# pirovc/ganon

Measured on AMD Instinct MI355X. Metric: Mreads/s classified (150 bp) + IBF-lookup GB/s vs HBM roofline, higher is better.
Workload: dtype u64

## Files before the change

### ganon_amd/build.py

```python
from __future__ import annotations

import os
import shutil
import subprocess
import sys

HERE = os.path.dirname(os.path.abspath(__file__))
ROOT = os.path.dirname(HERE)
CSRC = os.path.join(HERE, "csrc")
HOST = os.path.join(HERE, "host")
LIB = os.path.join(CSRC, "libganon_hip.so")
BIN = os.path.join(HOST, "ganon-classify")
BIN_BUILD = os.path.join(HOST, "ganon-build")
BIN_REASSIGN = os.path.join(HOST, "ganon-reassign")
BUILD_SHARED = ("seq_io.cpp", "pgzip.cpp", "filter_io.cpp")
REASSIGN_ONLY = ("reassign.cpp", "reassign_main.cpp")

HIP_SOURCES = ["gn_kernels.hip", "gn_split.hip", "gn_minimiser_lpr.hip", "gn_hibf.hip", "gn_postfilter.hip", "gn_build.hip", "gn_build_hibf.hip", "gn_build_sketch.hip", "gn_gather.hip", "gn_fastq.hip", "gn_reassign.hip", "gn_inflate.hip", "gn_capi.hip"]
HIP_HEADERS = ["gn_internal.h", "gn_devmem.h", "gn_scan.h", "gn_build_row.h", "gn_bin_spans.h", "gn_fold_table.h", "gn_screen_table.h", "gn_emplace_window.h", "gn_packed_set.h", "gn_path_window.h", os.path.join(ROOT, "include", "ganon_hip.h"), os.path.join(ROOT, "include", "ganon_ibf_hash.h")]


def _hipcc() -> str:
    for c in (shutil.which("hipcc"), "/opt/rocm/bin/hipcc"):
        if c and os.path.exists(c):
            return c
    raise RuntimeError("hipcc not found: libganon_hip.so cannot be built (there is no CPU fallback)")


def _stale(target: str, deps) -> bool:
    if not os.path.exists(target):
        return True
    t = os.path.getmtime(target)
    return any(os.path.getmtime(d) > t for d in deps if os.path.exists(d))


def build_hip(force: bool = False, verbose: bool = False) -> str:
    import concurrent.futures as cf
    hdrs = [h if os.path.isabs(h) else os.path.join(CSRC, h) for h in HIP_HEADERS]
    objdir = os.path.join(CSRC, "_obj")
    os.makedirs(objdir, exist_ok=True)
    hipcc = None
    jobs, objs = [], []
    for s in HIP_SOURCES:
        src = os.path.join(CSRC, s)
        obj = os.path.join(objdir, os.path.splitext(s)[0] + ".o")
        objs.append(obj)
        if force or _stale(obj, [src] + hdrs):
            hipcc = hipcc or _hipcc()
            jobs.append([hipcc, "--offload-arch=gfx950", "-O3", "-std=c++17", "-fPIC", "-Wno-unused-result", "-Wno-unused-value",
                         "-c", src, "-o", obj])

    def run(cmd):
# ... 43 lines not shown
```

### ganon_amd/csrc/gn_capi.hip

```cpp
#include "gn_internal.h"

#include <hipcub/hipcub.hpp>
#include "gn_scan.h"
#include "gn_screen_table.h"

#include <algorithm>
#include <cstdarg>
#include <cstdio>
#include <cstdlib>
#include <cstring>
#include <mutex>
#include <new>
#include <unordered_map>
#include <vector>

#include <sys/mman.h>

static thread_local char g_err[512] = "";

int gn_fail(int code, const char* fmt, ...)
{
    va_list ap;
    va_start(ap, fmt);
    vsnprintf(g_err, sizeof(g_err), fmt, ap);
    va_end(ap);
    return code;
}

extern "C" const char* gn_last_error(void)
{
    return g_err;
}

static GnSwitches g_sw;

static int gn_parse_switches(const char* list, GnSwitches* out, char* bad, size_t bad_len)
{
    GnSwitches sw;
    struct
    {
        const char* name;
        bool GnSwitches::* flag;
    } static const flags[] = {{"early_exit", &GnSwitches::early_exit},       {"row_screen", &GnSwitches::row_screen},       {"lean_screen", &GnSwitches::lean_screen},     {"cand_select", &GnSwitches::cand_select},
                              {"csr_identity", &GnSwitches::csr_identity},   {"uniform_select", &GnSwitches::uniform_select},
                              {"run_select", &GnSwitches::run_select},       {"max_first", &GnSwitches::max_first},
                              {"const_nb", &GnSwitches::const_nb},           {"split_kernel", &GnSwitches::split_kernel},
                              {"predrop", &GnSwitches::predrop},             {"deferred_grids", &GnSwitches::deferred_grids}, {"on_demand", &GnSwitches::on_demand}, {"hibf_dense_rows", &GnSwitches::hibf_dense_rows},
                              {"hibf_reg", &GnSwitches::hibf_reg},           {"hibf_pack", &GnSwitches::hibf_pack},
                              {"hibf_one_pack", &GnSwitches::hibf_one_pack}, {"gather_copy", &GnSwitches::gather_copy},     {"joint_apart", &GnSwitches::joint_apart},
                              {"pinned_malloc", &GnSwitches::pinned_malloc}, {"inflate_ahead", &GnSwitches::inflate_ahead}, {"debug", &GnSwitches::debug},
                              {"fake_count", &GnSwitches::fake_count}, {"seg_result", &GnSwitches::seg_result}};
    for (const char* p = list ? list : ""; *p;)
    {
        const char* e = strchr(p, ',');
        size_t      n = e ? (size_t)(e - p) : strlen(p);
        while (n && (*p == ' ' || *p == '\t'))
            ++p, --n;
        while (n && (p[n - 1] == ' ' || p[n - 1] == '\t'))
            --n;
        bool known = n == 0;
        for (const auto& f : flags)
            if (!known && strlen(f.name) == n && !strncmp(p, f.name, n))
                sw.*(f.flag) = true, known = true;
        if (!known && n > 6 && !strncmp(p, "chunk=", 6))
            sw.chunk = (uint32_t)strtoul(p + 6, nullptr, 10), known = true;
        if (!known && n > 11 && !strncmp(p, "emit_probe=", 11))
            sw.emit_probe = (uint32_t)strtoul(p + 11, nullptr, 10) & (64u | 128u), known = true;
        if (!known && n > 16 && !strncmp(p, "hibf_pair_limit=", 16))
            sw.hibf_pair_limit = std::max<uint64_t>(64, strtoull(p + 16, nullptr, 10)), known = true;
        if (!known && n > 5 && !strncmp(p, "sync=", 5))
        {
            const char* m = p + 5;
            const size_t l = n - 5;
            sw.sync_mode = (l == 4 && !strncmp(m, "spin", 4)) ? 1 : (l == 5 && !strncmp(m, "yield", 5)) ? 2 : (l == 5 && !strncmp(m, "block", 5)) ? 3 : -1;
            known = sw.sync_mode > 0;
        }
// ... 1144 lines not shown
    p.hashes     = s->v_hashes;
    p.slot_off   = s->v_slot_off;
    p.n_hashes   = s->v_nh;
    p.status     = s->v_status;
    p.n_reads    = hi;
    p.read_begin = lo;
    p.rel_cutoff = s->rel_cutoff;
    if (gn_sw().fake_count)
    {
        if (lo == 0)
            s->pf_predrop = false;
        if ((uint64_t)(hi + 1) / 2 <= s->match_cap && hi > lo)
            hipLaunchKernelGGL(gn_fake_count_kernel, dim3((hi - lo + 255) / 256), dim3(256), 0, s->st, s->d_matches, s->d_seg_begin, s->d_seg_count,
                               s->v_status, s->v_nh, lo, hi, (uint32_t)f->geom.wpr, f->n_targets ? f->n_targets : 1u, s->d_ctr);
        GN_HIP(hipGetLastError());
        return GN_OK;
    }
    p.wpr        = f->geom.wpr;
    p.gp_log2    = f->geom.gp_log2;
    p.slice_dwords = f->geom.slice_dwords;
    p.matches    = s->d_matches;
    p.match_cap  = s->match_cap;
    p.cursor     = s->d_ctr;
    p.seg_begin  = s->d_seg_begin;
    p.seg_count  = s->d_seg_count;
    p.dense      = nullptr;
    p.max_blocks = (uint32_t)f->n_cu * 16u;
    p.max_blocks_fast = (uint32_t)f->n_cu * (f->geom.lw == 1 ? 8u : 6u);
    p.max_blocks_lean = (uint32_t)f->n_cu * 10u;
    p.max_blocks_list = p.max_blocks_fast;
    p.emit_probe = gn_sw().emit_probe;
    p.early_exit = gn_sw().early_exit ? 0u : 1u;
    p.skip_ctr   = s->d_ctr + 7;
    if (f->identity && p.early_exit && !gn_sw().row_screen && (f->geom.lw == 1 || p.W > 128))
    {
        uint8_t ds[GN_SCREEN_NMAX + 1];
        gn_screen_table(p.rel_cutoff, f->ibf.h, (uint32_t)std::min<uint64_t>(f->ibf.W, 64u * f->geom.lw) * 64u, ds);
        memcpy(p.screen, ds, sizeof(p.screen));
    }
    if (lo == 0)
        GN_HIP(hipMemsetAsync(s->d_ctr + 7, 0, sizeof(unsigned long long), s->st));
    p.sl_nbr = f->d_sl_nbr;
    p.csr_identity = f->csr_identity && !gn_sw().csr_identity ? 1u : 0u;
    p.uniform_nb   = p.csr_identity && !gn_sw().uniform_select ? f->uniform_nb : 0u;
    p.run_select   = p.csr_identity && f->run_ok && !p.uniform_nb && !gn_sw().run_select ? 1u : 0u;
    p.max_first    = gn_sw().max_first ? 0u : 1u;
    p.const_nb     = p.uniform_nb && !gn_sw().const_nb ? p.uniform_nb : (p.run_select ? 4u : 0u);
    const bool split = !f->identity && f->d_sl_nbr != nullptr && !gn_sw().split_kernel;
    const bool fast = f->identity;
    const bool predrop = (fast || split) && s->pf_on && !s->pf_merge && s->pf.d_segmin && s->pf_rel_filter >= 0.0 && s->pf_rel_filter < 1.0 &&
                         (uint64_t)hi * f->geom.wpr <= s->pf.segmin_cap && !gn_sw().predrop;
    if (lo == 0)
        s->pf_predrop = predrop;
    if (predrop)
    {
        if (lo == 0)
            GN_HIP(hipMemsetAsync(s->pf.d_pre, 0, sizeof(unsigned long long), s->st));
        GN_HIP(hipMemsetAsync(s->pf.d_segmin + (size_t)lo * f->geom.wpr, 0xFF, (size_t)(hi - lo) * f->geom.wpr * 4, s->st));
        p.pre_mode = s->pf_joint ? 2u : 1u;
        p.pre_rel  = s->pf_rel_filter;
        p.seg_min  = s->pf.d_segmin;
        p.pre_ctr  = s->pf.d_pre;
    }
    if (split)
    {
        GN_HIP(hipMemsetAsync(s->d_ctr + 4, 0, sizeof(unsigned long long), s->st));
// ... 640 lines not shown
```

### ganon_amd/csrc/gn_internal.h

```cpp
#pragma once

#include <hip/hip_runtime.h>
#include <stdint.h>

#include <vector>

#include "../../include/ganon_hip.h"
#include "../../include/ganon_ibf_hash.h"
#include "gn_devmem.h"
#include "gn_packed_set.h"

#define GN_MAX_CHUNKS 64
#define GN_CAND_NBIG 4u
#define GN_HIBF_MAXDEPTH 64
#define GN_HIBF_TIMED_LEVELS 8
#define GN_PF_MAX_JOINT 16
#define GN_PF_MAX_DEVICES 16
#define GN_LONG_BLOCKS 128u
#define GN_NCTR 74

struct GnSwitches
{
    bool early_exit = false;
    bool row_screen = false;
    bool lean_screen = false;
    bool cand_select = false;
    bool csr_identity = false;
    bool uniform_select = false;
    bool run_select = false;
    bool max_first = false;
    bool const_nb = false;
    bool split_kernel = false;
    bool predrop = false;
    bool deferred_grids = false;
    bool seg_result = false;
    bool on_demand = false;
    bool hibf_reg = false;
    bool hibf_pack = false;
    bool hibf_one_pack = false;
    bool hibf_dense_rows = false;
    bool     inflate_ahead = false;
    uint64_t hibf_pair_limit = 0;
    bool gather_copy = false;
    bool joint_apart = false;
    uint32_t chunk = 0;
    int      sync_mode = 0;
    bool     pinned_malloc = false;
    bool     debug = false;
    uint32_t emit_probe = 0;
    bool     fake_count = false;
};
const GnSwitches& gn_sw();
struct gn_stream;
int             gn_result_compact(gn_stream* s);
const gn_match* gn_result_matches(gn_stream* s);

struct GnMinimiserParams
{
// ... 41 lines not shown
    uint32_t wpr;
    uint32_t gp_log2;
    uint32_t slice_dwords;
    gn_match*           matches;
    uint64_t            match_cap;
    unsigned long long* cursor;
    uint64_t*           seg_begin;
    uint32_t*           seg_count;
    uint16_t* dense;
    uint32_t  dense_begin, dense_end;
    const uint32_t*           work_list;
    const unsigned long long* work_count;
    uint32_t*                 work_list_out;
    unsigned long long*       work_count_out;
    const uint32_t*           unit_list;
    const unsigned long long* unit_count;
    uint32_t*                 unit_list_out;
    unsigned long long*       unit_count_out;
    uint32_t                  max_blocks_lean;
    uint32_t                  max_blocks_list;
    uint32_t                  max_blocks;
    uint32_t                  max_blocks_fast;
    uint32_t                  emit_probe;
    const uint32_t*           bin_tgt;
    const uint32_t*           bin_nb2;
    uint32_t                  nbtab_off;
    uint32_t                  candcnt_off;
    const uint32_t*           big_list;
    uint32_t                  n_big;
    const uint32_t*           sl_nbr;
    uint32_t                  early_exit;
    unsigned long long*       skip_ctr;
    uint32_t                  screen[32];
    unsigned long long*       grab;
    uint32_t            uniform_nb;
    uint32_t            max_first;
    uint32_t            const_nb;
    uint32_t            run_select;
    uint32_t            csr_identity;
    uint32_t            pre_mode;
    double              pre_rel;
    uint32_t*           seg_min;
    unsigned long long* pre_ctr;
};

__device__ __forceinline__ uint32_t gn_pf_threshold(uint32_t mx, uint32_t mn, double rel_filter)
{
    return mx - (uint32_t)(unsigned long long)ceil(__dmul_rn((double)(mx - mn), rel_filter));
}

struct GnCountGeometry
{
    uint32_t lw;
    uint32_t wpr;
    uint32_t gp_log2;
    uint32_t block;
    uint32_t rpb;
    uint32_t slice_dwords;
    size_t   lds_bytes;
    size_t   nbtab_off;
    size_t   candcnt_off;
};

bool gn_count_geometry(uint64_t W, uint32_t hash_funs, GnCountGeometry* g, const char** why);
uint32_t gn_count_lds_index(const GnCountGeometry& g, uint32_t b);

// ... 269 lines not shown
```

### ganon_amd/csrc/gn_kernels.hip

```cpp
#include "gn_internal.h"
#include <cstdlib>

#define GN_WAVE 64
#define GN_CAND_LIMIT 128u
#ifndef GN_NARROW_MAX
#define GN_NARROW_MAX 4u
#endif
#define GN_MATCH_CHUNK 256u
#ifndef GN_MATCH_CHUNK_MAX
#define GN_MATCH_CHUNK_MAX 8192u
#endif
#define GN_STAGE_CAP 128u

struct GnRankLut
{
    uint8_t t[256];
    constexpr GnRankLut() : t{}
    {
        for (int i = 0; i < 256; ++i)
            t[i] = 0;
        t['C'] = t['c'] = 1;
        t['G'] = t['g'] = 2;
        t['T'] = t['t'] = t['U'] = t['u'] = 3;
        t['Y'] = t['y'] = 1;
        t['S'] = t['s'] = 1;
        t['K'] = t['k'] = 2;
        t['B'] = t['b'] = 1;
    }
};
__constant__ GnRankLut GN_RANK_LUT = GnRankLut();

__constant__ uint64_t GN_IBF_SEEDS[GN_IBF_MAX_HASH_FUNS] = GN_IBF_SEED_LIST;

__device__ __forceinline__ void gn_wave_lds_sync()
{
    __builtin_amdgcn_fence(__ATOMIC_RELEASE, "wavefront");
    __builtin_amdgcn_wave_barrier();
    __builtin_amdgcn_fence(__ATOMIC_ACQUIRE, "wavefront");
}

// ... 872 lines not shown
#ifndef GN_FAST_WPE_LW1
#define GN_FAST_WPE_LW1 4
#endif
#ifndef GN_FAST_WPE_LW2
#define GN_FAST_WPE_LW2 2
#endif
#ifndef GN_FAST_WPE_LW2_H4
#define GN_FAST_WPE_LW2_H4 3
#endif

constexpr uint32_t GN_FAST_EE_GP_LOG2 = 6;
static_assert((1u << GN_FAST_EE_GP_LOG2) == GN_WAVE, "the EE instances of the fast kernel: one hash group a wave");
template <int HF, int LW, bool EE, bool WIDE = false, bool SCRN = false>
__global__ __launch_bounds__(256) __attribute__((amdgpu_waves_per_eu(EE ? (LW == 1 ? GN_FAST_WPE_LW1 : (HF <= 4 && !WIDE ? GN_FAST_WPE_LW2_H4 : GN_FAST_WPE_LW2)) : 1))) void gn_ibf_count_fast_kernel(GnCountParams p)
{
    extern __shared__ __attribute__((aligned(16))) uint32_t gn_lds[];
    constexpr int      ND   = 2 * LW;
    constexpr int      HFP  = HF <= 4 ? 4 : 8;
    constexpr uint32_t NMAX = 127;
    constexpr bool     SCR  = SCRN && EE && HF == 4 && (LW == 1 || WIDE);
    static_assert(SCR == SCRN, "a screening instance: early exit, four hash functions, 8-byte lanes or the wide build");
    constexpr bool     LST  = EE && !SCRN && !WIDE && HF == 4 && LW == 1;

    const int      lane  = threadIdx.x & (GN_WAVE - 1);
    const int      wave  = __builtin_amdgcn_readfirstlane((int)(threadIdx.x >> 6));
    const uint32_t wpr   = p.wpr;
    const uint32_t gpl   = SCR ? GN_FAST_EE_GP_LOG2 : p.gp_log2;
    const uint32_t Gp    = 1u << gpl;
    const uint32_t H     = GN_WAVE >> gpl;
    const uint32_t gl    = lane & (Gp - 1);
    const uint32_t hsub  = lane >> gpl;
    uint32_t*      rowtab = gn_lds + (size_t)wave * 128 * HFP;
    uint32_t*      mlist  = gn_lds + (size_t)(blockDim.x >> 6) * 128 * HFP + (size_t)wave * GN_FAST_LIST;

    uint64_t       n_units = (uint64_t)(p.n_reads - p.read_begin) * wpr;
    if constexpr (LST)
        if (p.unit_list)
            n_units = *p.unit_count;
    const uint64_t stride  = (uint64_t)gridDim.x * (blockDim.x >> 6);
    uint64_t       unit    = (uint64_t)blockIdx.x * (blockDim.x >> 6) + wave;
    if (unit >= n_units)
        return;
    const bool     dyn      = p.grab != nullptr && n_units >= 64u * stride;
    const uint64_t dyn_from = stride * 16u;
    uint64_t       chunk_end = unit + 1;
    if (dyn)
    {
        unit *= 16u;
        chunk_end = unit + 16u;
    }
    unsigned long long g_next = 0;
    uint32_t           g_size = 16u;
    auto               ask    = [&](uint64_t from) {
        g_size = from < n_units - n_units / 4u ? 16u : (from < n_units - n_units / 16u ? 8u : 4u);
        if (lane == 0)
            g_next = atomicAdd(p.grab, (unsigned long long)g_size);
    };
    if (dyn)
        ask(unit);
    const uint32_t q0_c = (uint32_t)lane / HF, q1_c = ((uint32_t)lane + GN_WAVE) / HF;
    auto hash_of = [&](uint32_t& q0, uint32_t& q1) {
        if constexpr (!SCR)
        {
            q0 = q0_c;
            q1 = q1_c;
            return;
// ... 168 lines not shown
            const uint2 v = *reinterpret_cast<const uint2*>(ptr);
            R.m[i][0] = v.x;
            R.m[i][1] = v.y;
        }
    };
    bool scr = SCR && ds != 0;
    auto issue = [&](uint32_t it, GnRowRegs<HF, LW>& R) {
        uint32_t q = it * H + hsub;
        q          = q < n ? q : n - 1;
        uint32_t row[HF];
#pragma unroll
        for (int i = 0; i < HF; ++i)
        {
            uint32_t idx = q * HFP + (uint32_t)i;
            if constexpr (SCR)
            {
                const uint32_t qs = 2 * it + (uint32_t)(i >> 1) < ds ? 2 * it + (uint32_t)(i >> 1) : 2 * it;
                idx               = scr ? qs * HFP + (uint32_t)(i & 1) : idx;
            }
            row[i] = rowtab[idx];
        }
#pragma unroll
        for (int i = 0; i < HF; ++i)
            load_row(row[i], R, i);
    };
    auto consume = [&](const GnRowRegs<HF, LW>& R, uint32_t it) {
        if (SCR && scr)
        {
            const uint32_t on = col_act ? 0xFFFFFFFFu : 0u, on2 = 2 * it + 1 < ds ? on : 0u;
#pragma unroll
            for (int d = 0; d < ND; ++d)
            {
                const uint32_t a = R.m[0][d] & R.m[1][d] & on, b = R.m[2 % HF][d] & R.m[3 % HF][d] & on2;
#pragma unroll
                for (int j = 0; j < 4; ++j)
                    nib[d][j] += ((a >> j) & 0x11111111u) + ((b >> j) & 0x11111111u);
            }
            acc_n += 2;
            if (acc_n >= 14)
            {
                spill_nibbles();
                acc_n = 0;
            }
            return;
        }
        const uint32_t on = (col_act && it * H + hsub < n) ? 0xFFFFFFFFu : 0u;
#pragma unroll
        for (int d = 0; d < ND; ++d)
        {
            uint32_t a = R.m[0][d] & on;
#pragma unroll
            for (int i = 1; i < HF; ++i)
                a &= R.m[i][d];
#pragma unroll
            for (int j = 0; j < 4; ++j)
                nib[d][j] += (a >> j) & 0x11111111u;
        }
        if (++acc_n == 15)
        {
            spill_nibbles();
            acc_n = 0;
        }
    };
    uint32_t sm[ND];
#pragma unroll
    for (int d = 0; d < ND; ++d)
// ... 114 lines not shown
        scr_rows            = 2 * ds;
        const uint32_t left = survey(ds);
        if (left == 0)
            dead = true;
        else if (left <= GN_NARROW_MAX)
            finish = true;
        if (dead || finish)
            break;
        aborted = true;
#pragma unroll
        for (int d = 0; d < ND; ++d)
#pragma unroll
            for (int j = 0; j < 4; ++j)
            {
                byt[d][j][0] = 0;
                byt[d][j][1] = 0;
            }
        issue(0, A);
    }
    uint32_t narrow_loads = 0;
    if (EE && (narrow || (SCR && finish)))
    {
        constexpr uint32_t QPC = GN_WAVE / HF;
        uint64_t           grp = 0;
#pragma unroll
        for (uint32_t q = 0; q < QPC; ++q)
            grp |= 1ULL << (q * HF);
        const uint32_t l_q = (uint32_t)lane / HF, l_i = (uint32_t)lane - l_q * HF;
        const uint32_t q_from = SCR && finish ? 0u : fetched;
        uint32_t       any_sm = 0;
#pragma unroll
        for (int d = 0; d < ND; ++d)
            any_sm |= sm[d];
        uint64_t lm = __ballot(any_sm != 0);
        while (lm)
        {
            const int L = __builtin_ctzll(lm);
            lm &= lm - 1;
#pragma unroll
            for (int d = 0; d < ND; ++d)
            {
                uint32_t mb = (uint32_t)__builtin_amdgcn_readlane((int)sm[d], L);
                while (mb)
                {
                    const uint32_t bit = (uint32_t)__builtin_ctz(mb);
                    mb &= mb - 1;
                    const uint32_t tp   = 32u * d + bit;
                    const uint32_t word = slice * 64 * LW + (uint32_t)L * LW + (tp >> 6);
                    const uint32_t sh   = tp & 63u;
                    uint32_t       add  = 0;
                    uint32_t       q_known = 0;
                    uint32_t       q_to    = n;
                    bool           probe   = false;
                    if (SCR && finish)
                    {
                        uint32_t c2 = 0;
#pragma unroll
                        for (int j = 0; j < 4; ++j)
#pragma unroll
                            for (int pp = 0; pp < 2; ++pp)
                                if ((bit & 3u) == (uint32_t)j && ((bit >> 2) & 1u) == (uint32_t)pp)
                                    c2 = byt[d][j][pp];
                        c2      = ((uint32_t)__builtin_amdgcn_readlane((int)c2, L) >> (8u * (bit >> 3))) & 0xFFu;
                        q_known = ds;
                        if (c2 != ds)
                        {
                            probe = true;
                            q_to  = ds;
                        }
                    }
                    for (;;)
                    {
                        add = 0;
                        for (uint32_t q0 = q_from; q0 < q_to; q0 += 2 * QPC)
                        {
                            const uint32_t qa = q0 + l_q, qb = qa + QPC;
                            const bool     ina = l_q < QPC && qa < q_to, inb = l_q < QPC && qb < q_to;
                            uint64_t       wa = ~0ULL, wb = ~0ULL;
                            if (ina && !(SCR && l_i < 2 && qa < q_known))
                                wa = p.rows[(uint64_t)rowtab[qa * HFP + l_i] * p.W + word];
                            if (inb && !(SCR && l_i < 2 && qb < q_known))
                                wb = p.rows[(uint64_t)rowtab[qb * HFP + l_i] * p.W + word];
                            const uint64_t bma = __ballot(ina && ((wa >> sh) & 1ULL)), bmb = __ballot(inb && ((wb >> sh) & 1ULL));
                            uint64_t       alla = bma, allb = bmb;
#pragma unroll
                            for (int i = 1; i < HF; ++i)
                            {
                                alla &= bma >> i;
                                allb &= bmb >> i;
                            }
                            add += (uint32_t)__popcll(alla & grp) + (uint32_t)__popcll(allb & grp);
                        }
                        narrow_loads += (q_to - q_from) * HF - 2 * q_known;
                        if (!(SCR && probe))
                            break;
                        probe = false;
                        if (add + (n - ds) < T)
                        {
                            add = 0;
                            break;
                        }
                        q_known = 0;
                        q_to    = n;
                    }
                    const uint32_t inc  = add << (8u * (bit >> 3));
                    const uint32_t keep = SCR && finish ? ~(0xFFu << (8u * (bit >> 3))) : 0xFFFFFFFFu;
#pragma unroll
                    for (int j = 0; j < 4; ++j)
#pragma unroll
                        for (int pp = 0; pp < 2; ++pp)
                            if ((bit & 3u) == (uint32_t)j && ((bit >> 2) & 1u) == (uint32_t)pp && lane == L)
                                byt[d][j][pp] = (byt[d][j][pp] & keep) + inc;
                }
            }
        }
    }
    if (slice * 64 * LW < p.W)
    {
        const uint32_t wcol = p.W - slice * 64 * LW < 64u * LW ? p.W - slice * 64 * LW : 64u * LW;
        if constexpr (!SCR)
        {
            if (dead || narrow)
            {
                const uint32_t got  = fetched < n ? fetched : n;
                const uint64_t full = (uint64_t)(n - got) * HF * wcol * 8ull;
                const uint64_t part = (uint64_t)narrow_loads * 128ull;
                skipped_bytes += full - part;
            }
        }
        else if (dead || narrow || finish)
        {
            const uint32_t got  = fetched < n ? fetched : n;
            const uint32_t rows = SCR && scr_rows && !aborted ? scr_rows : got * HF;
            const uint64_t full = (uint64_t)(n * HF - rows) * wcol * 8ull;
            const uint64_t part = (uint64_t)narrow_loads * 128ull;
// ... 251 lines not shown
        p.seg_begin[(size_t)read * wpr + slice] = base;
        p.seg_count[(size_t)read * wpr + slice] = total;
    }
    if (!more)
        break;
    unit = unit_n; read = read_n; n = n_n; slot = slot_n; hA = hA_n; hB = hB_n;
    }
    if (lane == 0 && skipped_bytes)
        atomicAdd(p.skip_ctr, (unsigned long long)skipped_bytes);
    if (p.pre_mode)
    {
#pragma unroll
        for (int off = 32; off > 0; off >>= 1)
            n_pre += (uint32_t)__shfl_xor((int)n_pre, off);
        if (lane == 0 && n_pre)
            atomicAdd(p.pre_ctr, (unsigned long long)n_pre);
    }
}

#ifndef GN_FAST_WPE_LEAN
#define GN_FAST_WPE_LEAN 5
#endif
__global__ __launch_bounds__(256) __attribute__((amdgpu_waves_per_eu(GN_FAST_WPE_LEAN))) void gn_ibf_count_fast_kernel_lean(GnCountParams p)
{
    extern __shared__ __attribute__((aligned(16))) uint32_t gn_lds[];
    constexpr int      HF   = 4;
    constexpr int      ND   = 2;
    constexpr uint32_t NMAX = 127;

    const int      lane   = threadIdx.x & (GN_WAVE - 1);
    const int      wave   = __builtin_amdgcn_readfirstlane((int)(threadIdx.x >> 6));
    const uint32_t wpr    = p.wpr;
    uint32_t*      rowtab = gn_lds + (size_t)wave * 128 * HF;

    const uint64_t n_units = (uint64_t)(p.n_reads - p.read_begin) * wpr;
    const uint64_t stride  = (uint64_t)gridDim.x * (blockDim.x >> 6);
    uint64_t       unit    = (uint64_t)blockIdx.x * (blockDim.x >> 6) + wave;
    if (unit >= n_units)
        return;
    const bool     dyn      = p.grab != nullptr && n_units >= 64u * stride;
    const uint64_t dyn_from = stride * 16u;
    uint64_t       chunk_end = unit + 1;
    if (dyn)
    {
        unit *= 16u;
        chunk_end = unit + 16u;
    }
    unsigned long long g_next = 0;
    uint32_t           g_size = 16u;
    auto               ask    = [&](uint64_t from) {
        g_size = from < n_units - n_units / 4u ? 16u : (from < n_units - n_units / 16u ? 8u : 4u);
        if (lane == 0)
            g_next = atomicAdd(p.grab, (unsigned long long)g_size);
    };
    if (dyn)
        ask(unit);
    auto hash_of = [&](uint32_t& q0, uint32_t& q1) {
        uint32_t l = (uint32_t)lane;
        asm volatile("" : "+v"(l));
        q0 = l / HF;
        q1 = (l + GN_WAVE) / HF;
    };
    auto load_meta = [&](uint64_t u, uint32_t& rd, uint32_t& nn, uint64_t& so) {
        uint32_t w = wpr;
        asm volatile("" : "+s"(w));
        rd = p.read_begin + (uint32_t)(u / w);
// ... 118 lines not shown
#pragma unroll
        for (int d = 0; d < ND; ++d)
#pragma unroll
            for (int j = 0; j < 4; ++j)
            {
                byt[d][j][0] += nib[d][j] & 0x0F0F0F0Fu;
                byt[d][j][1] += (nib[d][j] >> 4) & 0x0F0F0F0Fu;
                nib[d][j] = 0;
            }
    };
    const uint32_t wi_ld = col_act ? wi : 0u;
    auto issue = [&](uint32_t it, GnRowRegs<HF, 1>& R) {
        uint32_t row[HF];
#pragma unroll
        for (int i = 0; i < HF; ++i)
        {
            const uint32_t qs = 2 * it + (uint32_t)(i >> 1) < ds ? 2 * it + (uint32_t)(i >> 1) : 2 * it;
            row[i]            = rowtab[qs * HF + (uint32_t)(i & 1)];
        }
#pragma unroll
        for (int i = 0; i < HF; ++i)
        {
            const uint2 v = *reinterpret_cast<const uint2*>(p.rows + ((uint64_t)row[i] * p.W + wi_ld));
            R.m[i][0] = v.x;
            R.m[i][1] = v.y;
        }
    };
    auto consume = [&](const GnRowRegs<HF, 1>& R, uint32_t it) {
        const uint32_t on = col_act ? 0xFFFFFFFFu : 0u, on2 = 2 * it + 1 < ds ? on : 0u;
#pragma unroll
        for (int d = 0; d < ND; ++d)
        {
            const uint32_t a = R.m[0][d] & R.m[1][d] & on, b = R.m[2][d] & R.m[3][d] & on2;
#pragma unroll
            for (int j = 0; j < 4; ++j)
                nib[d][j] += ((a >> j) & 0x11111111u) + ((b >> j) & 0x11111111u);
        }
        acc_n += 2;
        if (acc_n >= 14)
        {
            spill_nibbles();
            acc_n = 0;
        }
    };
    GnRowRegs<HF, 1> A, Bq;
    issue(0, A);
    if (more)
        load_meta(unit_n, read_n, n_n, slot_n);
    {
        const uint32_t its = (ds + 1) >> 1;
        uint32_t       it  = 0;
        for (; it + 2 < its; it += 2)
        {
            issue(it + 1, Bq);
            consume(A, it);
            issue(it + 2, A);
            consume(Bq, it + 1);
        }
        const bool two = it + 1 < its;
        if (two)
            issue(it + 1, Bq);
        consume(A, it);
        if (two)
            consume(Bq, it + 1);
    }
    if (acc_n)
// ... 23 lines not shown
            uint32_t c = 0;
#pragma unroll
            for (int d = 0; d < ND; ++d)
                c += (uint32_t)__popc(sm[d]);
            for (int off = 32; off > 0; off >>= 1)
                c += __shfl_xor(c, off);
            left = (uint32_t)__builtin_amdgcn_readfirstlane((int)c);
        }
    }
    const uint32_t wcol = slice * 64 < p.W ? (p.W - slice * 64 < 64u ? p.W - slice * 64 : 64u) : 0u;
    if (more)
        load_hashes(n_n, slot_n, hA_n, hB_n);
    if (left > GN_NARROW_MAX)
    {
        if (lane == 0)
            p.unit_list_out[atomicAdd(p.unit_count_out, 1ULL)] = (uint32_t)unit;
        skipped_bytes -= (uint64_t)(2 * ds) * wcol * 8ull;
        if (!more)
            break;
        unit = unit_n; read = read_n; n = n_n; slot = slot_n; hA = hA_n; hB = hB_n;
        continue;
    }
    uint32_t narrow_loads = 0;
    uint32_t total = 0;
    uint32_t rec_t = 0, rec_c = 0;
    if (left)
    {
        constexpr uint32_t QPC = GN_WAVE / HF;
        uint64_t           grp = 0;
#pragma unroll
        for (uint32_t q = 0; q < QPC; ++q)
            grp |= 1ULL << (q * HF);
        const uint32_t l_q = (uint32_t)lane / HF, l_i = (uint32_t)lane - l_q * HF;
        uint64_t       lm  = __ballot((sm[0] | sm[1]) != 0);
        while (lm)
        {
            const int L = __builtin_ctzll(lm);
            lm &= lm - 1;
#pragma unroll
            for (int d = 0; d < ND; ++d)
            {
                uint32_t mb = (uint32_t)__builtin_amdgcn_readlane((int)sm[d], L);
                while (mb)
                {
                    const uint32_t bit = (uint32_t)__builtin_ctz(mb);
                    mb &= mb - 1;
                    const uint32_t word = slice * 64 + (uint32_t)L;
                    const uint32_t sh   = 32u * d + bit;
                    uint32_t       c2   = 0;
#pragma unroll
                    for (int j = 0; j < 4; ++j)
#pragma unroll
                        for (int pp = 0; pp < 2; ++pp)
                            if ((bit & 3u) == (uint32_t)j && ((bit >> 2) & 1u) == (uint32_t)pp)
                                c2 = byt[d][j][pp];
                    c2 = ((uint32_t)__builtin_amdgcn_readlane((int)c2, L) >> (8u * (bit >> 3))) & 0xFFu;
                    uint32_t add     = 0;
                    uint32_t q_known = ds;
                    uint32_t q_to    = n;
                    bool     probe   = c2 != ds;
                    if (probe)
                        q_to = ds;
                    for (;;)
                    {
                        add = 0;
                        for (uint32_t q0 = 0; q0 < q_to; q0 += 2 * QPC)
                        {
                            const uint32_t qa = q0 + l_q, qb = qa + QPC;
                            const bool     ina = qa < q_to, inb = qb < q_to;
                            uint64_t       wa = ~0ULL, wb = ~0ULL;
                            if (ina && !(l_i < 2 && qa < q_known))
                                wa = p.rows[(uint64_t)rowtab[qa * HF + l_i] * p.W + word];
                            if (inb && !(l_i < 2 && qb < q_known))
                                wb = p.rows[(uint64_t)rowtab[qb * HF + l_i] * p.W + word];
                            const uint64_t bma = __ballot(ina && ((wa >> sh) & 1ULL)), bmb = __ballot(inb && ((wb >> sh) & 1ULL));
                            uint64_t       alla = bma, allb = bmb;
#pragma unroll
                            for (int i = 1; i < HF; ++i)
                            {
                                alla &= bma >> i;
                                allb &= bmb >> i;
                            }
                            add += (uint32_t)__popcll(alla & grp) + (uint32_t)__popcll(allb & grp);
                        }
                        narrow_loads += q_to * HF - 2 * q_known;
                        if (!probe)
                            break;
                        probe = false;
                        if (add + (n - ds) < T)
                        {
                            add = 0;
                            break;
                        }
                        q_known = 0;
                        q_to    = n;
                    }
                    if (add >= T)
                    {
                        if ((uint32_t)lane == total)
                        {
                            rec_t = word * 64u + sh;
                            rec_c = add;
                        }
                        ++total;
                    }
                }
            }
        }
    }
    if (wcol)
        skipped_bytes += (uint64_t)(n * HF - 2 * ds) * wcol * 8ull - (uint64_t)narrow_loads * 128ull;

    unsigned long long base = 0;
    if (total)
    {
        if (total > chunk_left)
        {
            const uint32_t need = total > chunk_size ? total : chunk_size;
            chunk_size = chunk_size * 2u <= GN_MATCH_CHUNK_MAX ? chunk_size * 2u : GN_MATCH_CHUNK_MAX;
            unsigned long long nb = 0;
            if (lane == 0)
                nb = atomicAdd(p.cursor, (unsigned long long)need);
            chunk_base = gn_readlane64(nb, 0);
            chunk_left = need;
        }
        base = chunk_base;
        chunk_base += total;
        chunk_left -= total;
// ... 12 lines not shown
    {
        p.seg_begin[(size_t)read * wpr + slice] = base;
        p.seg_count[(size_t)read * wpr + slice] = total;
    }
    if (!more)
        break;
    unit = unit_n; read = read_n; n = n_n; slot = slot_n; hA = hA_n; hB = hB_n;
    }
    if (lane == 0 && skipped_bytes)
        atomicAdd(p.skip_ctr, (unsigned long long)skipped_bytes);
}

template <int HF, int LW, int MAXT>
static hipError_t gn_launch_count_one(const GnCountParams& p, const GnCountGeometry& g, hipStream_t st)
{
    uint32_t blocks = (p.n_reads - p.read_begin + g.rpb - 1) / g.rpb;
    if (blocks > p.max_blocks)
        blocks = p.max_blocks;
    (void)hipFuncSetAttribute(reinterpret_cast<const void*>(gn_ibf_count_kernel<HF, LW, MAXT>),
                              hipFuncAttributeMaxDynamicSharedMemorySize, (int)g.lds_bytes);
    hipLaunchKernelGGL((gn_ibf_count_kernel<HF, LW, MAXT>), dim3(blocks), dim3(g.block), g.lds_bytes, st, p);
    return hipGetLastError();
}

template <int HF, int LW>
static hipError_t gn_launch_fast_one(const GnCountParams& p, hipStream_t st)
{
    const bool ee = p.early_exit && p.gp_log2 == GN_FAST_EE_GP_LOG2;
    const uint64_t units  = (uint64_t)(p.n_reads - p.read_begin) * p.wpr;
    uint32_t       blocks = (uint32_t)((units + 3) / 4);
    if (blocks > p.max_blocks_fast)
        blocks = p.max_blocks_fast;
    const size_t   lds    = 4 * (128 * (HF <= 4 ? 4 : 8) + GN_FAST_LIST) * 4;
    bool scr = false;
    if constexpr (HF == 4)
        for (uint32_t w : p.screen)
            scr = scr || w != 0;
    scr = scr && ee;
    if constexpr (HF == 4 && LW == 2)
        if (scr && p.W > 128)
        {
            hipLaunchKernelGGL((gn_ibf_count_fast_kernel<HF, LW, true, true, true>), dim3(blocks), dim3(256), lds, st, p);
            return hipGetLastError();
        }
    if constexpr (HF == 4 && LW == 1)
        if (scr && p.unit_list_out != nullptr)
        {
            uint32_t lean_blocks = (uint32_t)((units + 3) / 4);
            if (lean_blocks > p.max_blocks_lean)
                lean_blocks = p.max_blocks_lean;
            hipLaunchKernelGGL(gn_ibf_count_fast_kernel_lean, dim3(lean_blocks), dim3(256), 4 * 128 * HF * 4, st, p);
            hipError_t e = hipGetLastError();
            if (e != hipSuccess)
                return e;
            GnCountParams q = p;
            q.unit_list     = p.unit_list_out;
            q.unit_count    = p.unit_count_out;
            q.grab          = nullptr;
            if (blocks > p.max_blocks_list)
                blocks = p.max_blocks_list;
            hipLaunchKernelGGL((gn_ibf_count_fast_kernel<HF, LW, true>), dim3(blocks ? blocks : 1u), dim3(256), lds, st, q);
            return hipGetLastError();
        }
    if constexpr (HF == 4 && LW == 1)
        if (scr)
        {
            hipLaunchKernelGGL((gn_ibf_count_fast_kernel<HF, LW, true, false, true>), dim3(blocks), dim3(256), lds, st, p);
            return hipGetLastError();
        }
    if (ee && LW == 2 && p.W > 128)
        hipLaunchKernelGGL((gn_ibf_count_fast_kernel<HF, LW, true, LW == 2>), dim3(blocks), dim3(256), lds, st, p);
    else if (ee)
        hipLaunchKernelGGL((gn_ibf_count_fast_kernel<HF, LW, true>), dim3(blocks), dim3(256), lds, st, p);
    else
        hipLaunchKernelGGL((gn_ibf_count_fast_kernel<HF, LW, false>), dim3(blocks), dim3(256), lds, st, p);
    return hipGetLastError();
}

hipError_t gn_launch_count_fast(const GnCountParams& p, const GnCountGeometry& g, uint32_t hash_funs, hipStream_t st)
{
    if (p.n_reads <= p.read_begin)
        return hipSuccess;
    const bool two = g.lw == 2;
    switch (hash_funs)
    {
        case 1: return two ? gn_launch_fast_one<1, 2>(p, st) : gn_launch_fast_one<1, 1>(p, st);
        case 2: return two ? gn_launch_fast_one<2, 2>(p, st) : gn_launch_fast_one<2, 1>(p, st);
        case 3: return two ? gn_launch_fast_one<3, 2>(p, st) : gn_launch_fast_one<3, 1>(p, st);
        case 4: return two ? gn_launch_fast_one<4, 2>(p, st) : gn_launch_fast_one<4, 1>(p, st);
        case 5: return two ? gn_launch_fast_one<5, 2>(p, st) : gn_launch_fast_one<5, 1>(p, st);
        default: return hipErrorInvalidValue;
    }
}

template <int HF>
static hipError_t gn_launch_count_hf(const GnCountParams& p, const GnCountGeometry& g, hipStream_t st)
{
    if (g.block <= 256)
        return g.lw == 2 ? gn_launch_count_one<HF, 2, 256>(p, g, st) : gn_launch_count_one<HF, 1, 256>(p, g, st);
    if (g.block <= 512)
// ... 164 lines not shown
```

Measured before the change: 265.2.

## Cache screen pair masks in LDS to probe-drop stray candidates early

During the screened pass, the kernel saves the per-lane two-hash AND masks for the first few screen iterations into LDS. When a candidate's screen count disagrees with the expected count, it uses those masks to load only the remaining hash words for the first hashes. It then derives an upper bound and drops the candidate before the full narrow re-probe. This trades extra LDS per wave (reducing occupancy headroom), an added wave-level LDS sync, and more code in the hot loop for fewer global row loads on stray candidates. A switch is added to disable it.

```diff
diff --git a/ganon_amd/build.py b/ganon_amd/build.py
--- a/ganon_amd/build.py
+++ b/ganon_amd/build.py
@@ -17,7 +17,7 @@
 REASSIGN_ONLY = ("reassign.cpp", "reassign_main.cpp")
 
 HIP_SOURCES = ["gn_kernels.hip", "gn_split.hip", "gn_minimiser_lpr.hip", "gn_hibf.hip", "gn_postfilter.hip", "gn_build.hip", "gn_build_hibf.hip", "gn_build_sketch.hip", "gn_gather.hip", "gn_fastq.hip", "gn_reassign.hip", "gn_inflate.hip", "gn_capi.hip"]
-HIP_HEADERS = ["gn_internal.h", "gn_devmem.h", "gn_scan.h", "gn_build_row.h", "gn_bin_spans.h", "gn_fold_table.h", "gn_screen_table.h", "gn_emplace_window.h", "gn_packed_set.h", "gn_path_window.h", os.path.join(ROOT, "include", "ganon_hip.h"), os.path.join(ROOT, "include", "ganon_ibf_hash.h")]
+HIP_HEADERS = ["gn_internal.h", "gn_devmem.h", "gn_scan.h", "gn_build_row.h", "gn_bin_spans.h", "gn_fold_table.h", "gn_screen_table.h", "gn_stray_probe.h", "gn_emplace_window.h", "gn_packed_set.h", "gn_path_window.h", os.path.join(ROOT, "include", "ganon_hip.h"), os.path.join(ROOT, "include", "ganon_ibf_hash.h")]
 
 
 def _hipcc() -> str:
diff --git a/ganon_amd/csrc/gn_capi.hip b/ganon_amd/csrc/gn_capi.hip
--- a/ganon_amd/csrc/gn_capi.hip
+++ b/ganon_amd/csrc/gn_capi.hip
@@ -3,6 +3,7 @@
 #include <hipcub/hipcub.hpp>
 #include "gn_scan.h"
 #include "gn_screen_table.h"
+#include "gn_stray_probe.h"
 
 #include <algorithm>
 #include <cstdarg>
@@ -41,7 +42,7 @@
     {
         const char* name;
         bool GnSwitches::* flag;
-    } static const flags[] = {{"early_exit", &GnSwitches::early_exit},       {"row_screen", &GnSwitches::row_screen},       {"lean_screen", &GnSwitches::lean_screen},     {"cand_select", &GnSwitches::cand_select},
+    } static const flags[] = {{"early_exit", &GnSwitches::early_exit},       {"row_screen", &GnSwitches::row_screen},       {"lean_screen", &GnSwitches::lean_screen},     {"stray_masks", &GnSwitches::stray_masks},     {"cand_select", &GnSwitches::cand_select},
                               {"csr_identity", &GnSwitches::csr_identity},   {"uniform_select", &GnSwitches::uniform_select},
                               {"run_select", &GnSwitches::run_select},       {"max_first", &GnSwitches::max_first},
                               {"const_nb", &GnSwitches::const_nb},           {"split_kernel", &GnSwitches::split_kernel},
@@ -1252,6 +1253,7 @@
     p.emit_probe = gn_sw().emit_probe;
     p.early_exit = gn_sw().early_exit ? 0u : 1u;
     p.skip_ctr   = s->d_ctr + 7;
+    p.probe_hashes = gn_sw().stray_masks ? 0u : GN_PROBE_HASHES;
     if (f->identity && p.early_exit && !gn_sw().row_screen && (f->geom.lw == 1 || p.W > 128))
     {
         uint8_t ds[GN_SCREEN_NMAX + 1];
diff --git a/ganon_amd/csrc/gn_internal.h b/ganon_amd/csrc/gn_internal.h
--- a/ganon_amd/csrc/gn_internal.h
+++ b/ganon_amd/csrc/gn_internal.h
@@ -24,6 +24,7 @@
     bool early_exit = false;
     bool row_screen = false;
     bool lean_screen = false;
+    bool stray_masks = false;
     bool cand_select = false;
     bool csr_identity = false;
     bool uniform_select = false;
@@ -131,6 +132,7 @@
     uint32_t                  early_exit;
     unsigned long long*       skip_ctr;
     uint32_t                  screen[32];
+    uint32_t                  probe_hashes;
     unsigned long long*       grab;
     uint32_t            uniform_nb;
     uint32_t            max_first;
diff --git a/ganon_amd/csrc/gn_kernels.hip b/ganon_amd/csrc/gn_kernels.hip
--- a/ganon_amd/csrc/gn_kernels.hip
+++ b/ganon_amd/csrc/gn_kernels.hip
@@ -6,6 +6,8 @@
 #ifndef GN_NARROW_MAX
 #define GN_NARROW_MAX 4u
 #endif
+#include "gn_stray_probe.h"
+static_assert(GN_PROBE_HASHES % 2u == 0 && GN_PROBE_HASHES * 4u <= GN_WAVE, "whole screen iterations (two hashes each), and stage 1 is one load a lane");
 #define GN_MATCH_CHUNK 256u
 #ifndef GN_MATCH_CHUNK_MAX
 #define GN_MATCH_CHUNK_MAX 8192u
@@ -944,6 +946,7 @@
     const uint32_t hsub  = lane >> gpl;
     uint32_t*      rowtab = gn_lds + (size_t)wave * 128 * HFP;
     uint32_t*      mlist  = gn_lds + (size_t)(blockDim.x >> 6) * 128 * HFP + (size_t)wave * GN_FAST_LIST;
+    uint32_t*      pmask  = gn_lds + (size_t)(blockDim.x >> 6) * (128 * HFP + GN_FAST_LIST) + (size_t)wave * (GN_PROBE_HASHES * ND * GN_WAVE);
 
     uint64_t       n_units = (uint64_t)(p.n_reads - p.read_begin) * wpr;
     if constexpr (LST)
@@ -1178,6 +1181,11 @@
             for (int d = 0; d < ND; ++d)
             {
                 const uint32_t a = R.m[0][d] & R.m[1][d] & on, b = R.m[2 % HF][d] & R.m[3 % HF][d] & on2;
+                if (2 * it < GN_PROBE_HASHES)
+                {
+                    pmask[((2 * it) * ND + (uint32_t)d) * GN_WAVE + (uint32_t)lane]     = a;
+                    pmask[((2 * it + 1) * ND + (uint32_t)d) * GN_WAVE + (uint32_t)lane] = b;
+                }
 #pragma unroll
                 for (int j = 0; j < 4; ++j)
                     nib[d][j] += ((a >> j) & 0x11111111u) + ((b >> j) & 0x11111111u);
@@ -1358,6 +1366,8 @@
 #pragma unroll
         for (int d = 0; d < ND; ++d)
             any_sm |= sm[d];
+        if constexpr (SCR)
+            gn_wave_lds_sync();
         uint64_t lm = __ballot(any_sm != 0);
         while (lm)
         {
@@ -1375,30 +1385,48 @@
                     const uint32_t word = slice * 64 * LW + (uint32_t)L * LW + (tp >> 6);
                     const uint32_t sh   = tp & 63u;
                     uint32_t       add  = 0;
+                    uint32_t       q_lo    = q_from;
                     uint32_t       q_known = 0;
                     uint32_t       q_to    = n;
                     bool           probe   = false;
-                    if (SCR && finish)
-                    {
-                        uint32_t c2 = 0;
-#pragma unroll
-                        for (int j = 0; j < 4; ++j)
-#pragma unroll
-                            for (int pp = 0; pp < 2; ++pp)
-                                if ((bit & 3u) == (uint32_t)j && ((bit >> 2) & 1u) == (uint32_t)pp)
-                                    c2 = byt[d][j][pp];
-                        c2      = ((uint32_t)__builtin_amdgcn_readlane((int)c2, L) >> (8u * (bit >> 3))) & 0xFFu;
-                        q_known = ds;
-                        if (c2 != ds)
+                    bool           dropped = false;
+                    uint32_t       e1      = 0;
+                    if constexpr (SCR)
+                        if (finish)
                         {
-                            probe = true;
-                            q_to  = ds;
+                            uint32_t c2 = 0;
+#pragma unroll
+                            for (int j = 0; j < 4; ++j)
+#pragma unroll
+                                for (int pp = 0; pp < 2; ++pp)
+                                    if ((bit & 3u) == (uint32_t)j && ((bit >> 2) & 1u) == (uint32_t)pp)
+                                        c2 = byt[d][j][pp];
+                            c2      = ((uint32_t)__builtin_amdgcn_readlane((int)c2, L) >> (8u * (bit >> 3))) & 0xFFu;
+                            q_known = ds;
+                            if (c2 != ds)
+                            {
+                                const uint32_t Fp   = gn_probe_first(p.probe_hashes, ds);
+                                bool           hitq = false;
+                                if (l_q < Fp)
+                                    hitq = ((pmask[(l_q * ND + (uint32_t)d) * GN_WAVE + (uint32_t)L] >> bit) & 1u) != 0;
+                                const bool ld = hitq && l_i >= 2;
+                                uint64_t   w1 = 0;
+                                if (ld)
+                                    w1 = p.rows[(uint64_t)rowtab[l_q * HFP + l_i] * p.W + word];
+                                const uint64_t hb = __ballot(ld && ((w1 >> sh) & 1ULL));
+                                const uint32_t m  = (uint32_t)__popcll(__ballot(hitq && l_i == 2));
+                                e1                = (uint32_t)__popcll(hb & (hb >> 1) & (grp << 2));
+                                narrow_loads += 2 * m;
+                                dropped = gn_probe_drop1(n, T, ds, c2, m, e1);
+                                probe = true;
+                                q_lo  = Fp;
+                                q_to  = ds;
+                            }
                         }
-                    }
-                    for (;;)
+                    while (!dropped)
                     {
                         add = 0;
-                        for (uint32_t q0 = q_from; q0 < q_to; q0 += 2 * QPC)
+                        for (uint32_t q0 = q_lo; q0 < q_to; q0 += 2 * QPC)
                         {
                             const uint32_t qa = q0 + l_q, qb = qa + QPC;
                             const bool     ina = l_q < QPC && qa < q_to, inb = l_q < QPC && qb < q_to;
@@ -1417,16 +1445,18 @@
                             }
                             add += (uint32_t)__popcll(alla & grp) + (uint32_t)__popcll(allb & grp);
                         }
-                        narrow_loads += (q_to - q_from) * HF - 2 * q_known;
+                        narrow_loads += (q_to - q_lo) * HF - 2 * (q_known - (SCR && probe ? q_lo : 0u));
                         if (!(SCR && probe))
                             break;
                         probe = false;
-                        if (add + (n - ds) < T)
+                        add += e1;
+                        if (gn_probe_drop2(n, T, ds, add))
                         {
                             add = 0;
                             break;
                         }
                         q_known = 0;
+                        q_lo    = 0;
                         q_to    = n;
                     }
                     const uint32_t inc  = add << (8u * (bit >> 3));
@@ -1744,6 +1774,7 @@
     const int      wave   = __builtin_amdgcn_readfirstlane((int)(threadIdx.x >> 6));
     const uint32_t wpr    = p.wpr;
     uint32_t*      rowtab = gn_lds + (size_t)wave * 128 * HF;
+    uint32_t*      pmask  = gn_lds + (size_t)(blockDim.x >> 6) * 128 * HF + (size_t)wave * (GN_PROBE_HASHES * ND * GN_WAVE);
 
     const uint64_t n_units = (uint64_t)(p.n_reads - p.read_begin) * wpr;
     const uint64_t stride  = (uint64_t)gridDim.x * (blockDim.x >> 6);
@@ -1928,6 +1959,13 @@
         for (int d = 0; d < ND; ++d)
         {
             const uint32_t a = R.m[0][d] & R.m[1][d] & on, b = R.m[2][d] & R.m[3][d] & on2;
+            if (2 * it < GN_PROBE_HASHES)
+            {
+                uint32_t l = (uint32_t)lane;
+                asm volatile("" : "+v"(l));
+                pmask[((2 * it) * ND + (uint32_t)d) * GN_WAVE + l]     = a;
+                pmask[((2 * it + 1) * ND + (uint32_t)d) * GN_WAVE + l] = b;
+            }
 #pragma unroll
             for (int j = 0; j < 4; ++j)
                 nib[d][j] += ((a >> j) & 0x11111111u) + ((b >> j) & 0x11111111u);
@@ -2017,6 +2055,8 @@
         for (uint32_t q = 0; q < QPC; ++q)
             grp |= 1ULL << (q * HF);
         const uint32_t l_q = (uint32_t)lane / HF, l_i = (uint32_t)lane - l_q * HF;
+        const uint32_t n_f = n, ds_f = ds;
+        gn_wave_lds_sync();
         uint64_t       lm  = __ballot((sm[0] | sm[1]) != 0);
         while (lm)
         {
@@ -2041,15 +2081,34 @@
                                 c2 = byt[d][j][pp];
                     c2 = ((uint32_t)__builtin_amdgcn_readlane((int)c2, L) >> (8u * (bit >> 3))) & 0xFFu;
                     uint32_t add     = 0;
-                    uint32_t q_known = ds;
-                    uint32_t q_to    = n;
+                    uint32_t q_lo    = 0;
+                    uint32_t q_known = ds_f;
+                    uint32_t q_to    = n_f;
                     bool     probe   = c2 != ds;
+                    bool     dropped = false;
+                    uint32_t e1      = 0;
                     if (probe)
-                        q_to = ds;
-                    for (;;)
+                    {
+                        const uint32_t Fp   = gn_probe_first(p.probe_hashes, ds);
+                        bool           hitq = false;
+                        if (l_q < Fp)
+                            hitq = ((pmask[(l_q * ND + (uint32_t)d) * GN_WAVE + (uint32_t)L] >> bit) & 1u) != 0;
+                        const bool ld = hitq && l_i >= 2;
+                        uint64_t   w1 = 0;
+                        if (ld)
+                            w1 = p.rows[(uint64_t)rowtab[l_q * HF + l_i] * p.W + word];
+                        const uint64_t hb = __ballot(ld && ((w1 >> sh) & 1ULL));
+                        const uint32_t m  = (uint32_t)__popcll(__ballot(hitq && l_i == 2));
+                        e1                = (uint32_t)__popcll(hb & (hb >> 1) & (grp << 2));
+                        narrow_loads += 2 * m;
+                        dropped = gn_probe_drop1(n, T, ds, c2, m, e1);
+                        q_lo    = Fp;
+                        q_to    = ds_f;
+                    }
+                    while (!dropped)
                     {
                         add = 0;
-                        for (uint32_t q0 = 0; q0 < q_to; q0 += 2 * QPC)
+                        for (uint32_t q0 = q_lo; q0 < q_to; q0 += 2 * QPC)
                         {
                             const uint32_t qa = q0 + l_q, qb = qa + QPC;
                             const bool     ina = qa < q_to, inb = qb < q_to;
@@ -2068,17 +2127,19 @@
                             }
                             add += (uint32_t)__popcll(alla & grp) + (uint32_t)__popcll(allb & grp);
                         }
-                        narrow_loads += q_to * HF - 2 * q_known;
+                        narrow_loads += (q_to - q_lo) * HF - 2 * (q_known - (probe ? q_lo : 0u));
                         if (!probe)
                             break;
                         probe = false;
-                        if (add + (n - ds) < T)
+                        add += e1;
+                        if (gn_probe_drop2(n, T, ds, add))
                         {
                             add = 0;
                             break;
                         }
                         q_known = 0;
-                        q_to    = n;
+                        q_lo    = 0;
+                        q_to    = n_f;
                     }
                     if (add >= T)
                     {
@@ -2157,6 +2218,7 @@
     if (blocks > p.max_blocks_fast)
         blocks = p.max_blocks_fast;
     const size_t   lds    = 4 * (128 * (HF <= 4 ? 4 : 8) + GN_FAST_LIST) * 4;
+    const size_t   lds_pm = 4 * (GN_PROBE_HASHES * 2 * LW * GN_WAVE) * 4;
     bool scr = false;
     if constexpr (HF == 4)
         for (uint32_t w : p.screen)
@@ -2165,7 +2227,7 @@
     if constexpr (HF == 4 && LW == 2)
         if (scr && p.W > 128)
         {
-            hipLaunchKernelGGL((gn_ibf_count_fast_kernel<HF, LW, true, true, true>), dim3(blocks), dim3(256), lds, st, p);
+            hipLaunchKernelGGL((gn_ibf_count_fast_kernel<HF, LW, true, true, true>), dim3(blocks), dim3(256), lds + lds_pm, st, p);
             return hipGetLastError();
         }
     if constexpr (HF == 4 && LW == 1)
@@ -2174,7 +2236,7 @@
             uint32_t lean_blocks = (uint32_t)((units + 3) / 4);
             if (lean_blocks > p.max_blocks_lean)
                 lean_blocks = p.max_blocks_lean;
-            hipLaunchKernelGGL(gn_ibf_count_fast_kernel_lean, dim3(lean_blocks), dim3(256), 4 * 128 * HF * 4, st, p);
+            hipLaunchKernelGGL(gn_ibf_count_fast_kernel_lean, dim3(lean_blocks), dim3(256), 4 * (128 * HF + GN_PROBE_HASHES * 2 * GN_WAVE) * 4, st, p);
             hipError_t e = hipGetLastError();
             if (e != hipSuccess)
                 return e;
@@ -2190,7 +2252,7 @@
     if constexpr (HF == 4 && LW == 1)
         if (scr)
         {
-            hipLaunchKernelGGL((gn_ibf_count_fast_kernel<HF, LW, true, false, true>), dim3(blocks), dim3(256), lds, st, p);
+            hipLaunchKernelGGL((gn_ibf_count_fast_kernel<HF, LW, true, false, true>), dim3(blocks), dim3(256), lds + lds_pm, st, p);
             return hipGetLastError();
         }
     if (ee && LW == 2 && p.W > 128)
diff --git a/ganon_amd/csrc/gn_stray_probe.h b/ganon_amd/csrc/gn_stray_probe.h
--- /dev/null
+++ b/ganon_amd/csrc/gn_stray_probe.h
@@ -0,0 +1,27 @@
+#pragma once
+#include <cstdint>
+
+#ifndef GN_PROBE_HASHES
+#define GN_PROBE_HASHES 4u
+#endif
+
+#if defined(__HIPCC__) || defined(__CUDACC__)
+#define GN_PROBE_HD __host__ __device__ inline
+#else
+#define GN_PROBE_HD inline
+#endif
+
+GN_PROBE_HD uint32_t gn_probe_first(uint32_t F, uint32_t ds)
+{
+    return F < ds ? F : ds;
+}
+
+GN_PROBE_HD bool gn_probe_drop1(uint32_t n, uint32_t T, uint32_t ds, uint32_t c2, uint32_t m, uint32_t e)
+{
+    return e + (c2 - m) + (n - ds) < T;
+}
+
+GN_PROBE_HD bool gn_probe_drop2(uint32_t n, uint32_t T, uint32_t ds, uint32_t add)
+{
+    return add + (n - ds) < T;
+}
```

After: 275.9 (median of 6 runs). +4.0%, better.
